# elador/FeatureDetection

Hardware: AMD Instinct MI355X
Metric: Mpatches/s (extract+WVM+SVM) per GPU, 640x480 pyramid (higher is better)
Workload: dtype u8/i32/f32/f64; 1 GPU; config 1/metric config: ffpDetectApp FaceFrontal.cfg five-stage cascade on 640x480 BGR frames: 13-layer pyramid, 20x20 windows step 1 (16185 windows/frame), HistEq64 -> WVM 280 filters -> OE -> RBF-SVM 1024 SV -> NMS; fd_pyramid_update_frames + fd_detect_five_stage_frames (the frames of a call share one pyramid aren...; frames_per_call=64, calls_in_flight=11, parallelism=image-shard dp1

## Files before the change

### featuredetection_amd/csrc/pyramid.hip

```cpp
#include "fd_internal.hpp"
#include <algorithm>
#include <cstring>

namespace {

constexpr int MAXJ = 16;

struct ResizeJob {
    int dw, dh;
    uint32_t dst_off;
    double scale_x, scale_y;
};
struct ResizeJobs {
    int n;
    ResizeJob j[MAXJ];
};
struct DownJob {
    int sw, sh;
    uint32_t src_off, dst_off;
};
struct FusedJob {
    int dw0, dh0, dw1, dh1;
    uint32_t dst0_off;
    uint32_t dst1_off;
    uint32_t xtab;
    double scale_y;
};
struct FusedJobs {
    int n;
    FusedJob j[MAXJ];
};
struct DownJobs {
    int n;
    int tile0[MAXJ + 1];
    DownJob j[MAXJ];
};
struct FilterJob {
    int w, h;
    uint32_t src_off, dst_off;
};
struct FilterJobs {
    int n;
    FilterJob j[MAXJ];
};

__device__ __forceinline__ int reflect101(int p, int len) {
    if (len == 1) return 0;
    while (p < 0 || p >= len) {
        if (p < 0) p = -p;
        else p = 2 * len - 2 - p;
    }
    return p;
}
__device__ __forceinline__ int reflect1(int p, int len) {
    if (len < 3) return reflect101(p, len);
    const int q = p < 0 ? -p : (p >= len ? 2 * len - 2 - p : p);
    return min(max(q, 0), len - 1);
}

struct FramePtrs {
    const uint8_t* p[FD_MAX_FRAMES];
};
__device__ __forceinline__ unsigned int mul24(unsigned int a, unsigned int b) {
    unsigned int r;
    asm("v_mul_u32_u24 %0, %1, %2" : "=v"(r) : "v"(a), "v"(b));
    return r;
}
__device__ __forceinline__ unsigned int mul24_s(unsigned int a_uniform, unsigned int b) {
    unsigned int r;
    asm("v_mul_u32_u24 %0, %1, %2" : "=v"(r) : "s"(a_uniform), "v"(b));
    return r;
}
__device__ __forceinline__ unsigned int mad24(unsigned int a, unsigned int b, unsigned int c) {
    unsigned int r;
    asm("v_mad_u32_u24 %0, %1, %2, %3" : "=v"(r) : "v"(a), "v"(b), "v"(c));
    return r;
}
__device__ __forceinline__ unsigned int mulhi24(unsigned int a, unsigned int b) {
    unsigned int r;
    asm("v_mul_hi_u32_u24 %0, %1, %2" : "=v"(r) : "v"(a), "v"(b));
    return r;
}
typedef unsigned short u16x2 __attribute__((ext_vector_type(2)));
__device__ __forceinline__ uint32_t ld_u32_unaligned(const uint8_t* p) {
    uint32_t v;
    __builtin_memcpy(&v, p, 4);
    return v;
}
__device__ __forceinline__ uint32_t gray_of(uint32_t b, uint32_t g, uint32_t r) { return (b * 1868u + g * 9617u + r * 4899u + 8192u) >> 14; }

__global__ void k_frames_to_gray(FramePtrs frames, uint8_t* __restrict__ grayBase, size_t imageStride, int n, int ch) {
    const uint8_t* __restrict__ src = frames.p[blockIdx.y];
    uint8_t* __restrict__ gray = grayBase + (size_t)blockIdx.y * imageStride;
    const int nq = n >> 2;
    const bool aligned = ((uintptr_t)src & 3) == 0;
    const int stride = gridDim.x * blockDim.x;
    auto load3 = [&](int q, uint32_t (&w)[3]) {
        if (aligned) {
            const uint32_t* s3 = reinterpret_cast<const uint32_t*>(src) + 3 * (size_t)q;
            w[0] = s3[0]; w[1] = s3[1]; w[2] = s3[2];
        } else {
            const uint8_t* s1 = src + 12 * (size_t)q;
            w[0] = ld_u32_unaligned(s1); w[1] = ld_u32_unaligned(s1 + 4); w[2] = ld_u32_unaligned(s1 + 8);
        }
    };
    auto gray4 = [&](const uint32_t (&w)[3]) {
        const uint32_t g0 = gray_of(w[0] & 255u, (w[0] >> 8) & 255u, (w[0] >> 16) & 255u);
        const uint32_t g1 = gray_of(w[0] >> 24, w[1] & 255u, (w[1] >> 8) & 255u);
        const uint32_t g2 = gray_of((w[1] >> 16) & 255u, w[1] >> 24, w[2] & 255u);
        const uint32_t g3 = gray_of((w[2] >> 8) & 255u, (w[2] >> 16) & 255u, w[2] >> 24);
        return g0 | (g1 << 8) | (g2 << 16) | (g3 << 24);
    };
    constexpr int GQ = 4;
    for (int q = blockIdx.x * blockDim.x + threadIdx.x; q < nq; q += GQ * stride) {
        if (ch == 3) {
            uint32_t w[GQ][3];
#pragma unroll
            for (int i = 0; i < GQ; ++i) load3(min(q + i * stride, nq - 1), w[i]);
#pragma unroll
            for (int i = 0; i < GQ; ++i)
                if (q + i * stride < nq) reinterpret_cast<uint32_t*>(gray)[q + i * stride] = gray4(w[i]);
        } else {
            uint32_t w[GQ];
#pragma unroll
            for (int i = 0; i < GQ; ++i) w[i] = ld_u32_unaligned(src + 4 * (size_t)min(q + i * stride, nq - 1));
#pragma unroll
            for (int i = 0; i < GQ; ++i)
                if (q + i * stride < nq) reinterpret_cast<uint32_t*>(gray)[q + i * stride] = w[i];
        }
    }
    if (blockIdx.x == 0 && (int)threadIdx.x < (n & 3)) {
        const int i = (nq << 2) + threadIdx.x;
        gray[i] = ch == 3 ? (uint8_t)gray_of(src[3 * (size_t)i], src[3 * (size_t)i + 1], src[3 * (size_t)i + 2]) : src[i];
    }
}

__global__ void k_bgr2gray(const uint8_t* __restrict__ bgr, uint8_t* __restrict__ gray, int n) {
    int i = blockIdx.x * blockDim.x + threadIdx.x;
    int stride = gridDim.x * blockDim.x;
    for (; i < n; i += stride) {
        int b = bgr[3 * (size_t)i], g = bgr[3 * (size_t)i + 1], r = bgr[3 * (size_t)i + 2];
        gray[i] = (uint8_t)((b * 1868 + g * 9617 + r * 4899 + 8192) >> 14);
// ... 75 lines not shown
    __shared__ int4 rowTab[TL_H];
    const ResizeJob jb = jobs.j[blockIdx.y];
    const uint8_t* src = arena + (size_t)blockIdx.z * imageStride + src_off;
    uint8_t* dst = out + (size_t)blockIdx.z * imageStride + jb.dst_off;
    const int tilesX = (jb.dw + TL_W - 1) / TL_W, tilesY = (jb.dh + TL_H - 1) / TL_H;
    auto srcX = [&](int dx, float& fx) {
        fx = (float)((dx + 0.5) * jb.scale_x - 0.5);
        int sx = (int)floorf(fx);
        fx -= sx;
        if (sx < 0) { fx = 0; sx = 0; }
        if (sx >= sw - 1) { fx = 0; sx = sw - 1; }
        return sx;
    };
    auto srcY = [&](int dy, float& fy) {
        fy = (float)((dy + 0.5) * jb.scale_y - 0.5);
        const int sy = (int)floorf(fy);
        fy -= sy;
        return sy;
    };
    auto clampY = [&](int y) { return y < 0 ? 0 : (y >= sh ? sh - 1 : y); };
    const int c = threadIdx.x & 63, rq = __builtin_amdgcn_readfirstlane(threadIdx.x >> 6);
    for (int t = blockIdx.x; t < tilesX * tilesY; t += gridDim.x) {
        const int ty = t / tilesX, tx = t - ty * tilesX;
        const int dx0 = tx * TL_W, dy0 = ty * TL_H;
        const int X0 = max(0, (int)((float)dx0 * (float)jb.scale_x) - 1), Y0 = max(0, (int)((float)dy0 * (float)jb.scale_y) - 1);
        {
            const int x = X0 + 4 * c;
            const bool colok = c < TL_PITCH / 4;
            uint32_t v[TL_ROWS / 4];
#pragma unroll
            for (int k = 0; k < TL_ROWS / 4; ++k) {
                const int sy = min(Y0 + rq + 4 * k, sh - 1);
                v[k] = 0;
                if (colok && x + 3 < sw) v[k] = ld_u32_unaligned(src + (uint32_t)(sy * sw) + x);
            }
            if (colok && x + 3 >= sw) {
#pragma unroll 1
                for (int k = 0; k < TL_ROWS / 4; ++k) {
                    const uint8_t* row = src + (uint32_t)(min(Y0 + rq + 4 * k, sh - 1) * sw);
                    uint32_t w = 0;
                    for (int b = 0; b < 4; ++b) w |= (uint32_t)row[min(x + b, sw - 1)] << (8 * b);
                    v[k] = w;
                }
            }
            if (colok) {
#pragma unroll
                for (int k = 0; k < TL_ROWS / 4; ++k) *reinterpret_cast<uint32_t*>(&tile[(rq + 4 * k) * TL_PITCH + 4 * c]) = v[k];
            }
        }
        if (threadIdx.x < TL_H) {
            float fy;
            const int sy = srcY(dy0 + threadIdx.x, fy);
            rowTab[threadIdx.x] = make_int4((clampY(sy) - Y0) * TL_PITCH, (clampY(sy + 1) - Y0) * TL_PITCH, __float2int_rn((1.f - fy) * 2048),
                                            __float2int_rn(fy * 2048));
        }
        __syncthreads();
        const int dx = dx0 + c;
        if (dx < jb.dw) {
            float fx;
            const int sx = srcX(dx, fx);
            const int a0 = __float2int_rn((1.f - fx) * 2048), a1 = __float2int_rn(fx * 2048);
            const int lx = sx - X0, lx1 = (sx + 1 < sw ? sx + 1 : sx) - X0;
            uint8_t* dp = dst + (uint32_t)((dy0 + rq * (TL_H / 4)) * jb.dw) + dx;
#pragma unroll
            for (int k = 0; k < TL_H / 4; ++k, dp += jb.dw) {
                const int rr = rq * (TL_H / 4) + k;
                if (dy0 + rr < jb.dh) {
                    const int4 rt = rowTab[rr];
                    const uint8_t* S0 = tile + rt.x;
                    const uint8_t* S1 = tile + rt.y;
                    const unsigned int r0 = __umul24(S0[lx], a0) + __umul24(S0[lx1], a1);
                    const unsigned int r1 = __umul24(S1[lx], a0) + __umul24(S1[lx1], a1);
                    *dp = (uint8_t)(((__umul24(rt.z, r0 >> 4) >> 16) + (__umul24(rt.w, r1 >> 4) >> 16) + 2) >> 2);
                }
            }
        }
        __syncthreads();
    }
}

#ifdef FD_PYR_PROF
constexpr int PYR_PROF_WGS = 65536;
__device__ unsigned long long fd_pyr_prof[PYR_PROF_WGS * 8];
#define PYR_T(x) const unsigned long long x = __builtin_amdgcn_s_memtime()
#else
#define PYR_T(x)
#endif
constexpr int FT_W1 = 62, FT_H1 = 16;
constexpr int G0_W = 2 * FT_W1 + 3, G0_H = 2 * FT_H1 + 3, G0_PITCH = 128;
constexpr int FS_PITCH = 256;
constexpr int FS_LOADS = (2 * G0_H + 3) / 4;
struct FusedFetch {
    uint32_t v[FS_LOADS];
    int2 ex;
    uint32_t taps;
};
__device__ __forceinline__ void fused_issue(FusedFetch& f, const uint8_t* __restrict__ src, int sw, int sh, const int2* __restrict__ tabs,
                                            const FusedJob& jb, const int4 d) {
    const int X0 = d.x, ncol = d.y;
    const int gx0 = 2 * (d.z & 0xffff) * FT_W1 - 2, gy0 = 2 * (int)((uint32_t)d.z >> 16) * FT_H1 - 2;
    const int lane = threadIdx.x & 63, wave = __builtin_amdgcn_readfirstlane(threadIdx.x >> 6);
    uint32_t rowOff;
    {
        const int py = gy0 + min((wave >> 1) + 2 * lane, G0_H - 1), pr = py < 0 ? -py : (py >= jb.dh0 ? 2 * jb.dh0 - 2 - py : py);
        float fy = (float)((min(max(pr, 0), jb.dh0 - 1) + 0.5) * jb.scale_y - 0.5);
        const int sy = (int)floorf(fy);
        fy -= sy;
        f.taps = (uint32_t)__float2int_rn((1.f - fy) * 2048) | (uint32_t)__float2int_rn(fy * 2048) << 16;
        rowOff = mul24((uint32_t)min(max(sy + (wave & 1), 0), sh - 1), (uint32_t)sw);
    }
    const uint32_t voff = (uint32_t)(4 * min(lane, (ncol - 1) >> 2) + X0);
#pragma unroll
    for (int q = 0; q < FS_LOADS; ++q) f.v[q] = ld_u32_unaligned(src + ((uint32_t)__builtin_amdgcn_readlane((int)rowOff, q) + voff));
    f.ex = tabs[jb.xtab + reflect101(gx0 + (int)(threadIdx.x & 127), jb.dw0)];
}

__global__ __launch_bounds__(256) void k_resize_down(uint8_t* __restrict__ arena0, uint32_t src_off, int sw, int sh, const int2* __restrict__ tabs,
                                                     FusedJobs jobs, uint32_t tileTab, int tilesPerFrame, int nimg, size_t imageStride) {
    __shared__ __attribute__((aligned(16))) uint8_t stage[4 * FS_LOADS * FS_PITCH];
    __shared__ __attribute__((aligned(16))) uint8_t g0[G0_H * G0_PITCH];
    __shared__ uint2 taps[G0_H];
    const int4* tiles = reinterpret_cast<const int4*>(tabs + tileTab);
    const int lane = threadIdx.x & 63, wave = __builtin_amdgcn_readfirstlane(threadIdx.x >> 6);
    const bool byXcd = nimg >= 8 && (gridDim.x & 7u) == 0;
    const int xcd = blockIdx.x & 7;
    const int slot = byXcd ? (int)(blockIdx.x >> 3) : (int)blockIdx.x, nslot = byXcd ? (int)(gridDim.x >> 3) : (int)gridDim.x;
    const int items = (byXcd ? (nimg - xcd + 7) >> 3 : nimg) * tilesPerFrame;
    auto frame_of = [&](int item) { const int fi = item / tilesPerFrame; return byXcd ? xcd + 8 * fi : fi; };
    auto desc_of = [&](int item) { return item < items ? tiles[item % tilesPerFrame] : make_int4(0, 0, 0, 0); };

    int item = slot;
    if (item >= items) return;
    int4 d = desc_of(item);
    FusedFetch f;
    fused_issue(f, arena0 + (size_t)frame_of(item) * imageStride + src_off, sw, sh, tabs, jobs.j[d.w], d);
    int itemN = item + nslot;
    int4 dN = desc_of(itemN);

#ifdef FD_PYR_PROF
    unsigned long long pacc[6] = {0, 0, 0, 0, 0, 0}, ptiles = 0;
#endif
    for (; item < items; item = itemN, d = dN, itemN += nslot, dN = desc_of(itemN)) {
        PYR_T(p0);
        const FusedJob jb = jobs.j[d.w];
        uint8_t* arena = arena0 + (size_t)frame_of(item) * imageStride;
        const int X0 = d.x;
        const int x1 = (d.z & 0xffff) * FT_W1, y1 = (int)((uint32_t)d.z >> 16) * FT_H1;
        const int gx0 = 2 * x1 - 2, gy0 = 2 * y1 - 2;
        {
            static_assert(2 * G0_H <= 4 * FS_LOADS && FS_PITCH == 256, "stage holds a dword per lane for slots wave + 4 q");
#pragma unroll
            for (int q = 0; q < FS_LOADS; ++q) *reinterpret_cast<uint32_t*>(&stage[(wave + 4 * q) * FS_PITCH + 4 * lane]) = f.v[q];
            const int i = (wave >> 1) + 2 * lane;
            if ((wave & 1) == 0 && i < G0_H) taps[i] = make_uint2((f.taps & 0xffffu) << 12, (f.taps >> 16) << 12);
        }
        const int2 ex = f.ex;
        PYR_T(p1);
        __syncthreads();
        PYR_T(p2);
        if (itemN < items)
            fused_issue(f, arena0 + (size_t)frame_of(itemN) * imageStride + src_off, sw, sh, tabs, jobs.j[dN.w], dN);
        PYR_T(p3);
        {
            const int c = threadIdx.x & 127, half = __builtin_amdgcn_readfirstlane(threadIdx.x >> 7);
            if (c < G0_W) {
                const int rBase = half * (G0_H - 18);
                const int lx = min(max(ex.x - X0, 0), FS_PITCH - 1) + 2 * rBase * FS_PITCH;
                int lx1 = lx + 1;
                asm("" : "+v"(lx1));
                const uint8_t *sp = stage + lx, *sp1 = stage + lx1;
                const uint2* tp = taps + rBase;
                const u16x2 aw = __builtin_bit_cast(u16x2, ex.y);
                uint8_t* gp = g0 + rBase * G0_PITCH + c;
#pragma unroll
                for (int i = 0; i < 18; ++i) {
                    const uint8_t *s = sp + 2 * i * FS_PITCH, *s1 = sp1 + 2 * i * FS_PITCH;
                    const u16x2 p0 = {s[0], s1[0]}, p1 = {s[FS_PITCH], s1[FS_PITCH]};
                    const uint2 t = tp[i];
                    const unsigned int h0 = __builtin_amdgcn_udot2(p0, aw, 0u, false) & ~15u;
                    const unsigned int h1 = __builtin_amdgcn_udot2(p1, aw, 0u, false) & ~15u;
                    gp[i * G0_PITCH] = (uint8_t)((mulhi24(t.x, h0) + mulhi24(t.y, h1) + 2) >> 2);
                }
            }
        }
        PYR_T(p4);
        __syncthreads();
        PYR_T(p5);
        {
            const int c1 = lane;
            const int x = x1 + c1;
            if (c1 < FT_W1 && x < jb.dw1) {
                constexpr int PR = FT_H1 / 4;
                const uint8_t* T = g0 + (2 * wave * PR) * G0_PITCH + 2 * c1;
                int h[2 * PR + 3];
#pragma unroll
                for (int r = 0; r < 2 * PR + 3; ++r) {
                    const uint8_t* S = T + r * G0_PITCH;
                    const uint32_t p01 = *reinterpret_cast<const uint16_t*>(S), p23 = *reinterpret_cast<const uint16_t*>(S + 2);
                    h[r] = (int)__builtin_amdgcn_udot4(p01 | (p23 << 16), 0x04060401u, (uint32_t)S[4], false);
                }
                uint8_t* dp = arena + jb.dst1_off + (uint32_t)((y1 + wave * PR) * jb.dw1) + x;
#pragma unroll
                for (int j = 0; j < PR; ++j, dp += jb.dw1) {
                    if (y1 + wave * PR + j < jb.dh1) {
                        const int v = h[2 * j + 2] * 6 + (h[2 * j + 1] + h[2 * j + 3]) * 4 + h[2 * j] + h[2 * j + 4];
                        *dp = (uint8_t)((v + 128) >> 8);
                    }
                }
            }
        }
        if (jb.dst0_off != 0xffffffffu) {
            uint8_t* d0 = arena + jb.dst0_off;
            for (int i = threadIdx.x; i < 32 * 128; i += 256) {
                const int r = 2 + (i >> 7), c = 2 + (i & 127);
                const int gx = gx0 + c, gy = gy0 + r;
                if (c < 2 + 2 * FT_W1 && gx < jb.dw0 && gy < jb.dh0) d0[(uint32_t)(gy * jb.dw0) + gx] = g0[r * G0_PITCH + c];
            }
        }
#ifdef FD_PYR_PROF
        {
            const unsigned long long p6 = __builtin_amdgcn_s_memtime();
            pacc[0] += p1 - p0; pacc[1] += p2 - p1; pacc[2] += p3 - p2; pacc[3] += p4 - p3; pacc[4] += p5 - p4; pacc[5] += p6 - p5; ++ptiles;
        }
#endif
    }
#ifdef FD_PYR_PROF
    if (threadIdx.x == 0 && blockIdx.x < (unsigned int)PYR_PROF_WGS) {
        for (int i = 0; i < 6; ++i) fd_pyr_prof[blockIdx.x * 8 + i] = pacc[i];
        fd_pyr_prof[blockIdx.x * 8 + 6] = ptiles;
    }
#endif
}

__device__ __forceinline__ int reflect_cf(int p, int len) {
    int q = p < 0 ? -p : p;
    q = q >= len ? 2 * len - 2 - q : q;
    return min(max(q, 0), len - 1);
}
constexpr int PD_W = 62;
__global__ __launch_bounds__(256) void k_pyrdown_tiled(uint8_t* __restrict__ arena, DownJobs jobs, size_t imageStride) {
    __shared__ __attribute__((aligned(16))) uint8_t tile[TL_ROWS * TL_PITCH];
    arena += (size_t)blockIdx.z * imageStride;
    const int c = threadIdx.x & 63, rq = __builtin_amdgcn_readfirstlane(threadIdx.x >> 6);
    constexpr int NROWS = 2 * PD_TH + 3, PD_LD = (NROWS + 7) / 8;
    static_assert(2 * (3 + 4 * (PD_LD - 1)) + 1 < TL_ROWS && 128 <= TL_PITCH && 2 * PD_W + 3 <= 128, "pyrDown stage");
    for (int g = blockIdx.x; g < jobs.tile0[jobs.n]; g += gridDim.x) {
        int ji = 0;
        while (ji + 1 < jobs.n && g >= jobs.tile0[ji + 1]) ++ji;
        const DownJob jb = jobs.j[ji];
        const int t = g - jobs.tile0[ji];
        const int sw = jb.sw, sh = jb.sh;
        const int dw = (sw + 1) / 2, dh = (sh + 1) / 2;
        const uint8_t* src = arena + jb.src_off;
        uint8_t* dst = arena + jb.dst_off;
        const int tilesX = (dw + PD_W - 1) / PD_W;
        const int ty = t / tilesX, tx = t - ty * tilesX;
        const int dx0 = tx * PD_W, dy0 = ty * PD_TH;
        const int X0 = 2 * dx0 - 2, Y0 = 2 * dy0 - 2;
        {
            const int j4 = 4 * (c & 31), half = c >> 5;
            const int xs = X0 + j4;
            const int xc = min(max(xs, 0), max(sw - 4, 0));
            const uint32_t lastDw = (uint32_t)max(sw * sh - 4, 0);
            uint32_t v[PD_LD];
#pragma unroll
            for (int k = 0; k < PD_LD; ++k) {
                const int r = 2 * (rq + 4 * k) + half;
                v[k] = ld_u32_unaligned(src + min((uint32_t)(reflect_cf(Y0 + r, sh) * sw + xc), lastDw));
            }
            if (X0 < 0 || X0 + 128 > sw) {
                if (!(xs >= 0 && xs + 3 < sw)) {
#pragma unroll
                    for (int k = 0; k < PD_LD; ++k) {
                        const int r = 2 * (rq + 4 * k) + half;
                        const uint8_t* row = src + (uint32_t)(reflect_cf(Y0 + r, sh) * sw);
                        uint32_t w = 0;
#pragma unroll
                        for (int b = 0; b < 4; ++b) w |= (uint32_t)row[reflect_cf(xs + b, sw)] << (8 * b);
                        v[k] = w;
                    }
                }
            }
#pragma unroll
            for (int k = 0; k < PD_LD; ++k) *reinterpret_cast<uint32_t*>(&tile[(2 * (rq + 4 * k) + half) * TL_PITCH + j4]) = v[k];
        }
        __syncthreads();
        const int x = dx0 + c;
        if (c < PD_W && x < dw) {
            constexpr int PR = PD_TH / 4;
            const uint8_t* T = tile + (2 * rq * PR) * TL_PITCH + 2 * c;
            int h[2 * PR + 3];
#pragma unroll
            for (int r = 0; r < 2 * PR + 3; ++r) {
                const uint8_t* S = T + r * TL_PITCH;
                const uint32_t p01 = *reinterpret_cast<const uint16_t*>(S), p23 = *reinterpret_cast<const uint16_t*>(S + 2);
                h[r] = (int)__builtin_amdgcn_udot4(p01 | (p23 << 16), 0x04060401u, (uint32_t)S[4], false);
            }
            uint8_t* dp = dst + (uint32_t)((dy0 + rq * PR) * dw) + x;
#pragma unroll
            for (int j = 0; j < PR; ++j, dp += dw) {
                if (dy0 + rq * PR + j < dh) {
                    const int v = h[2 * j + 2] * 6 + (h[2 * j + 1] + h[2 * j + 3]) * 4 + h[2 * j] + h[2 * j + 4];
                    *dp = (uint8_t)((v + 128) >> 8);
                }
            }
        }
        __syncthreads();
    }
}

__device__ __forceinline__ float grad_pair(const uint8_t* __restrict__ src, int w, int h, int x, int y, int ksize, int& gx, int& gy) {
    if (ksize == 1 || ksize == 3) {
        const int xm = reflect101(x - 1, w), xp = reflect101(x + 1, w);
        const int ym = reflect101(y - 1, h), yp = reflect101(y + 1, h);
        const uint8_t *S0 = src + (size_t)ym * w, *S1 = src + (size_t)y * w, *S2 = src + (size_t)yp * w;
        if (ksize == 1) {
            gx = S1[xp] - S1[xm];
            gy = S2[x] - S0[x];
            return 0.5f;
        }
        gx = (S0[xp] - S0[xm]) + 2 * (S1[xp] - S1[xm]) + (S2[xp] - S2[xm]);
        gy = (S2[xm] - S0[xm]) + 2 * (S2[x] - S0[x]) + (S2[xp] - S0[xp]);
        return 0.125f;
    }
    int a, d1, d2, d3, s0, s1, s2, s3;
    float scale;
    if (ksize == 5) { a = 2; d1 = 2; d2 = 1; d3 = 0; s0 = 6; s1 = 4; s2 = 1; s3 = 0; scale = 1.f / 128.f; }
    else if (ksize == 7) { a = 3; d1 = 5; d2 = 4; d3 = 1; s0 = 20; s1 = 15; s2 = 6; s3 = 1; scale = 1.f / 2048.f; }
    else { a = 1; d1 = 1; d2 = 0; d3 = 0; s0 = 10; s1 = 3; s2 = 0; s3 = 0; scale = 1.f / 32.f; }
// ... 203 lines not shown
    __shared__ unsigned int lm[4][3];
#pragma unroll
    for (int c = 0; c < 3; ++c) {
        unsigned long long sc = s[c];
        unsigned int mc = m[c];
        for (int o = 32; o > 0; o >>= 1) {
            sc += __shfl_down(sc, o, 64);
            mc = max(mc, (unsigned int)__shfl_down((int)mc, o, 64));
        }
        if ((threadIdx.x & 63) == 0) { ls[threadIdx.x >> 6][c] = sc; lm[threadIdx.x >> 6][c] = mc; }
    }
    __syncthreads();
    if (threadIdx.x < 3) {
        const int c = threadIdx.x;
        atomicAdd(&stats[blockIdx.y].sum[c], ls[0][c] + ls[1][c] + ls[2][c] + ls[3][c]);
        atomicMax(&stats[blockIdx.y].max[c], max(max(lm[0][c], lm[1][c]), max(lm[2][c], lm[3][c])));
    }
}

__global__ __launch_bounds__(256) void k_gw_gray(FramePtrs frames, const GwStats* __restrict__ stats, uint8_t* __restrict__ grayBase,
                                                 size_t imageStride, int n) {
    __shared__ double scale[3];
    __shared__ uint32_t tab[3][256];
    const uint8_t* __restrict__ src = frames.p[blockIdx.y];
    uint8_t* __restrict__ gray = grayBase + (size_t)blockIdx.y * imageStride;
    const int nq = n >> 2;
    const bool aligned = ((uintptr_t)src & 3) == 0;
    const int stride = gridDim.x * blockDim.x;
    int q = blockIdx.x * blockDim.x + threadIdx.x;
    uint32_t w[GW_GQ][3] = {};
    if (q < nq) {
#pragma unroll
        for (int i = 0; i < GW_GQ; ++i) gw_load3(src, aligned, min(q + i * stride, nq - 1), w[i]);
    }
    if (threadIdx.x < 64) {
        const GwStats& S = stats[blockIdx.y];
        double mean[3], maxNew[3];
        for (int c = 0; c < 3; ++c) { mean[c] = (double)S.sum[c] / n; maxNew[c] = (uint8_t)S.max[c] / mean[c]; }
        double mx = maxNew[0];
        if (maxNew[1] > mx) mx = maxNew[1];
        if (maxNew[2] > mx) mx = maxNew[2];
        if (threadIdx.x == 0)
            for (int c = 0; c < 3; ++c) scale[c] = 255.0 / (mean[c] * mx);
    }
    __syncthreads();
    {
        const uint32_t v = threadIdx.x;
        const uint32_t wgt[3] = {1868u, 9617u, 4899u};
#pragma unroll
        for (int c = 0; c < 3; ++c) {
            const int r = __double2int_rn(scale[c] * (double)v);
            tab[c][v] = (uint32_t)min(255, max(0, r)) * wgt[c] + (c == 0 ? 8192u : 0u);
        }
    }
    __syncthreads();
    auto gray1 = [&](uint32_t b, uint32_t g, uint32_t r) { return (tab[0][b] + tab[1][g] + tab[2][r]) >> 14; };
    auto gray4 = [&](const uint32_t (&x)[3]) {
        const uint32_t g0 = gray1(x[0] & 255u, (x[0] >> 8) & 255u, (x[0] >> 16) & 255u);
        const uint32_t g1 = gray1(x[0] >> 24, x[1] & 255u, (x[1] >> 8) & 255u);
        const uint32_t g2 = gray1((x[1] >> 16) & 255u, x[1] >> 24, x[2] & 255u);
        const uint32_t g3 = gray1((x[2] >> 8) & 255u, (x[2] >> 16) & 255u, x[2] >> 24);
        return g0 | (g1 << 8) | (g2 << 16) | (g3 << 24);
    };
    while (q < nq) {
        const int qn = q + GW_GQ * stride;
        uint32_t wn[GW_GQ][3] = {};
        if (qn < nq) {
#pragma unroll
            for (int i = 0; i < GW_GQ; ++i) gw_load3(src, aligned, min(qn + i * stride, nq - 1), wn[i]);
        }
#pragma unroll
        for (int i = 0; i < GW_GQ; ++i)
            if (q + i * stride < nq) reinterpret_cast<uint32_t*>(gray)[q + i * stride] = gray4(w[i]);
#pragma unroll
        for (int i = 0; i < GW_GQ; ++i) { w[i][0] = wn[i][0]; w[i][1] = wn[i][1]; w[i][2] = wn[i][2]; }
        q = qn;
    }
    if (blockIdx.x == 0 && (int)threadIdx.x < (n & 3)) {
        const size_t i = ((size_t)nq << 2) + threadIdx.x;
        gray[i] = (uint8_t)gray1(src[3 * i], src[3 * i + 1], src[3 * i + 2]);
    }
}

inline uint32_t align256(size_t v) { return (uint32_t)((v + 255) & ~(size_t)255); }

void build_gradient_lut(int bins, bool signedGradients, bool interpolate, std::vector<uint8_t>& lut) {
    const double PI = 3.1415926535897932384626433832795;
    const int E = interpolate ? 4 : 2;
    lut.resize((size_t)65536 * E);
    for (int x = 0; x < 256; ++x) {
        double gradientX = ((double)x - 127) / 255;
        for (int y = 0; y < 256; ++y) {
            double gradientY = ((double)y - 127) / 255;
            double direction = std::atan2(gradientY, gradientX);
            double magnitude = std::sqrt(gradientX * gradientX + gradientY * gradientY);
            double bin;
            if (signedGradients) {
                direction += PI;
                bin = direction * bins / (2 * PI);
            } else {
                if (direction < 0) direction += PI;
                bin = direction * bins / PI;
            }
            auto sat = [](double v) { int r = fd_cvRound(v); return (uint8_t)(r < 0 ? 0 : (r > 255 ? 255 : r)); };
            size_t index = (size_t)x | ((size_t)y << 8);
            if (!interpolate) {
                lut[2 * index] = (uint8_t)((uint8_t)std::round(bin) % (unsigned)bins);
                lut[2 * index + 1] = sat(255 * magnitude);
            } else {
                uint8_t w1 = sat(255 * magnitude * (bin - std::floor(bin)));
                lut[4 * index] = (uint8_t)((uint8_t)std::floor(bin) % (unsigned)bins);
                lut[4 * index + 1] = sat(255 * magnitude - w1);
                lut[4 * index + 2] = (uint8_t)((uint8_t)std::ceil(bin) % (unsigned)bins);
                lut[4 * index + 3] = w1;
            }
        }
    }
}

void build_resize_tables(fd_pyramid* p, int W, int H) {
    p->rtab_x.assign(p->all.size(), ~0u);
    static const int mode = [] { const char* e = getenv("FD_PYR_FUSED"); return e ? atoi(e) : 1; }();
    if (mode == 0) return;
    std::vector<int2> tab;
    std::vector<std::vector<int4>> tiles;
    p->rtile_off.clear();
    p->rtile_cnt.clear();
    int nfused = 0;
    for (size_t k = 0; k + 1 < p->all.size(); ++k) {
        const HostLayer& L = p->all[k];
        const HostLayer& D = p->all[k + 1];
        if (L.depth != 0 || D.depth != 1 || D.chain != L.chain) continue;
        if (L.w == W && L.h == H && L.gray_off == p->gray_full_off) continue;
        if (L.w < 3 || L.h < 3 || W > 65535 || H > 65535) continue;
        if (L.kept && mode != 2) continue;
        const double scale_x = 1. / ((double)L.w / W);
        std::vector<int2> xt((size_t)L.w);
        for (int dx = 0; dx < L.w; ++dx) {
            float fx = (float)((dx + 0.5) * scale_x - 0.5);
            int sx = (int)floorf(fx);
            fx -= sx;
            if (sx < 0) { fx = 0; sx = 0; }
            if (sx >= W - 1) { fx = 0; sx = W - 1; }
            const int a0 = (int)nearbyintf((1.f - fx) * 2048), a1 = (int)nearbyintf(fx * 2048);
            xt[(size_t)dx] = make_int2(sx, a0 | (a1 << 16));
        }
        bool fits = true;
        for (int x1 = 0; x1 < D.w && fits; x1 += FT_W1) {
            const int cLo = std::max(0, 2 * x1 - 2), cHi = std::min(L.w - 1, 2 * x1 - 2 + G0_W - 1);
            fits = std::min(W - 1, xt[(size_t)cHi].x + 1) - xt[(size_t)cLo].x + 1 <= FS_PITCH;
        }
        if (!fits) continue;
        {
            if (nfused % MAXJ == 0) tiles.emplace_back();
            std::vector<int4>& tl = tiles.back();
            for (int ty = 0; ty * FT_H1 < D.h; ++ty)
                for (int tx = 0; tx * FT_W1 < D.w; ++tx) {
                    const int gx0 = 2 * tx * FT_W1 - 2;
                    const int cLo = std::max(0, gx0), cHi = std::min(L.w - 1, gx0 + G0_W - 1);
                    const int X0 = xt[(size_t)cLo].x, ncol = std::min(W - 1, xt[(size_t)cHi].x + 1) - X0 + 1;
                    tl.push_back(make_int4(X0, ncol, (int)((uint32_t)tx | (uint32_t)ty << 16), nfused % MAXJ));
                }
            ++nfused;
        }
        p->rtab_x[k] = (uint32_t)tab.size();
        tab.insert(tab.end(), xt.begin(), xt.end());
    }
    if (tab.empty()) return;
    for (const std::vector<int4>& tl : tiles) {
        if (tab.size() & 1) tab.push_back(make_int2(0, 0));
        p->rtile_off.push_back((uint32_t)tab.size());
        p->rtile_cnt.push_back((int)tl.size());
        for (const int4& t : tl) { tab.push_back(make_int2(t.x, t.y)); tab.push_back(make_int2(t.z, t.w)); }
    }
    p->rtab.reserve(sizeof(int2) * tab.size());
    HIP_CHECK(hipMemcpy(p->rtab.p, tab.data(), sizeof(int2) * tab.size(), hipMemcpyHostToDevice));
}

void build_layout(fd_pyramid* p, int W, int H) {
    p->img_w = W;
    p->img_h = H;
    p->all.clear();
    p->kept.clear();
    size_t off = 0;
    p->gray_full_off = 0;
    off = align256((size_t)W * H);
    const int fch = p->filter_kind == FD_LAYER_GRADBIN ? (p->interpolate ? 4 : 2) : 1;
    for (size_t i = 0; i < p->octl; ++i) {
        double scaleFactor = std::pow(p->inc, (double)i);
        int w = fd_cvRound(W * scaleFactor), h = fd_cvRound(H * scaleFactor);
        if (w < 1 || h < 1) FD_THROW(FD_ERR_INVALID_ARGUMENT, "ImagePyramid: layer %zu would be empty", i);
        int depth = 0;
        const bool isFull = (w == W && h == H);
        HostLayer L{(int)i, scaleFactor, w, h, 1, (uint32_t)(isFull ? p->gray_full_off : off), 0, scaleFactor <= p->maxS && scaleFactor >= p->minS, (int)i, depth};
        if (!isFull) off = align256(off + (size_t)w * h);
        p->all.push_back(L);
        int pw = w, ph = h;
        scaleFactor *= 0.5;
        for (size_t j = 1; scaleFactor >= p->minS && pw > 1; ++j, scaleFactor *= 0.5) {
            int dw = (pw + 1) / 2, dh = (ph + 1) / 2;
            HostLayer D{(int)(i + j * p->octl), scaleFactor, dw, dh, 1, (uint32_t)off, 0, scaleFactor <= p->maxS, (int)i, (int)j};
            off = align256(off + (size_t)dw * dh);
            p->all.push_back(D);
            pw = dw;
            ph = dh;
        }
    }
    for (size_t k = 0; k < p->all.size(); ++k) {
        HostLayer& L = p->all[k];
        if (!L.kept) continue;
        L.ch = fch;
        if (p->filter_kind == FD_LAYER_NONE) L.filt_off = L.gray_off;
        else {
            L.filt_off = (uint32_t)off;
            off = align256(off + (size_t)L.w * L.h * fch);
            if (p->filter_kind == FD_LAYER_GRADBIN && p->grad_blur > 0) {
                L.blur_off = (uint32_t)off;
                off = align256(off + (size_t)L.w * L.h);
            }
        }
        p->kept.push_back((int)k);
    }
    if (off > 0xfffffff0ull) FD_THROW(FD_ERR_INVALID_ARGUMENT, "ImagePyramid: pyramid exceeds 4 GB arena");
    std::sort(p->kept.begin(), p->kept.end(), [&](int a, int b) { return p->all[a].index < p->all[b].index; });
    p->arena_bytes = off + 256;
    p->image_stride = (p->arena_bytes + 255) & ~(size_t)255;
    if (p->nimg > 1 && p->image_stride * (size_t)p->nimg > 0xfffffff0ull * 16) FD_THROW(FD_ERR_INVALID_ARGUMENT, "ImagePyramid: multi-frame pyramid too large");
    p->arena.reserve(p->image_stride * (size_t)p->nimg);
    p->h_layer_table.clear();
    for (int k : p->kept) {
        const HostLayer& L = p->all[k];
        p->h_layer_table.push_back(LayerDesc{L.w, L.h, L.ch, 0, L.gray_off, L.filt_off});
    }
    p->layer_table.reserve(sizeof(LayerDesc) * std::max<size_t>(1, p->h_layer_table.size()));
    if (!p->h_layer_table.empty())
        HIP_CHECK(hipMemcpyAsync(p->layer_table.p, p->h_layer_table.data(), sizeof(LayerDesc) * p->h_layer_table.size(),
                                 hipMemcpyHostToDevice, p->ctx->stream));
    build_resize_tables(p, W, H);
}

int grid_for(int npix) { return std::max(1, std::min(1024, (npix + 255) / 256)); }
int tile_grid_for(int ntiles) { return std::max(1, std::min(1024, ntiles)); }

void pyramid_update(fd_pyramid* p, const uint8_t* image, int W, int H, int ch, int is_device, hipStream_t st, const uint8_t* const* frames = nullptr) {
    if (!image && !frames) FD_THROW(FD_ERR_INVALID_ARGUMENT, "fd_pyramid_update: image is NULL");
    if (p->nimg > 1 && !frames) FD_THROW(FD_ERR_INVALID_ARGUMENT, "fd_pyramid_update: the pyramid holds %d frames, use fd_pyramid_update_frames", p->nimg);
    if (p->nimg > 1 && p->filter_kind != FD_LAYER_NONE) FD_THROW(FD_ERR_INVALID_ARGUMENT, "multi-frame pyramids have no layer filters");
    if (W < 1 || H < 1) FD_THROW(FD_ERR_INVALID_ARGUMENT, "fd_pyramid_update: empty image");
    if (ch != 1 && ch != 3) FD_THROW(FD_ERR_INVALID_ARGUMENT, "fd_pyramid_update: image must have 1 or 3 channels");
    const bool greyworld = p->image_filter != FD_IMAGE_GRAY;
    if (greyworld && ch != 3) FD_THROW(FD_ERR_INVALID_ARGUMENT, "GreyWorldNormalizationFilter: The image type must be CV_8UC3");
    if (greyworld && (size_t)W * H > 0x7fffffffull) FD_THROW(FD_ERR_INVALID_ARGUMENT, "GreyWorldNormalizationFilter: image too large");
    if (W != p->img_w || H != p->img_h || p->all.empty()) build_layout(p, W, H);
    uint8_t* arena = p->arena.as<uint8_t>();
    const size_t npix = (size_t)W * H;
    const int NI = frames ? p->nimg : 1;
    const size_t IS = p->image_stride;
    auto enqueue_rest = [&]() {
    int maxDepth = 0;
    for (const HostLayer& L : p->all) maxDepth = std::max(maxDepth, L.depth);
    {
        ResizeJobs jobs;
        jobs.n = 0;
        int maxpix = 0, maxtiles = 0;
        auto flush = [&]() {
            if (!jobs.n) return;
            bool fits = true;
            for (int q = 0; q < jobs.n; ++q)
                fits = fits && jobs.j[q].scale_x >= 1.0 && jobs.j[q].scale_x <= 2.05 && jobs.j[q].scale_y >= 1.0 && jobs.j[q].scale_y <= 2.05;
            if (fits)
                hipLaunchKernelGGL(k_resize_tiled, dim3(tile_grid_for(maxtiles), jobs.n, NI), dim3(256), 0, st, arena, arena, p->gray_full_off, W, H, jobs, IS);
            else
                hipLaunchKernelGGL(k_resize_linear, dim3(grid_for(maxpix), jobs.n, NI), dim3(256), 0, st, arena, arena, p->gray_full_off, W, H, jobs, IS);
            jobs.n = 0;
            maxpix = 0;
            maxtiles = 0;
        };
        for (size_t k = 0; k < p->all.size(); ++k) {
            const HostLayer& L = p->all[k];
            if (L.depth != 0) continue;
            if (L.w == W && L.h == H && L.gray_off == p->gray_full_off) continue;
            if (p->rtab_x[k] != ~0u) continue;
            ResizeJob& j = jobs.j[jobs.n++];
            j.dw = L.w; j.dh = L.h; j.dst_off = L.gray_off;
            j.scale_x = 1. / ((double)L.w / W);
            j.scale_y = 1. / ((double)L.h / H);
            maxpix = std::max(maxpix, L.w * L.h);
            maxtiles = std::max(maxtiles, ((L.w + TL_W - 1) / TL_W) * ((L.h + TL_H - 1) / TL_H));
            if (jobs.n == MAXJ) flush();
        }
        flush();
    }
    {
        FusedJobs jobs;
        jobs.n = 0;
        size_t group = 0;
        auto flush = [&]() {
            if (!jobs.n) return;
            static int perCu = 0;
            if (perCu == 0 && (hipOccupancyMaxActiveBlocksPerMultiprocessor(&perCu, k_resize_down, 256, 0) != hipSuccess || perCu < 1)) perCu = 4;
            const int tilesPerFrame = p->rtile_cnt[group];
            int grid = (int)std::min<int64_t>((int64_t)tilesPerFrame * NI, (int64_t)p->ctx->num_cus * perCu);
            if (NI >= 8 && grid >= 64) grid &= ~7;
            hipLaunchKernelGGL(k_resize_down, dim3(grid), dim3(256), 0, st, arena, p->gray_full_off, W, H, p->rtab.as<int2>(), jobs, p->rtile_off[group], tilesPerFrame, NI, IS);
            jobs.n = 0;
            ++group;
        };
        for (size_t k = 0; k + 1 < p->all.size(); ++k) {
            if (p->rtab_x[k] == ~0u) continue;
            const HostLayer& L = p->all[k];
            const HostLayer& D = p->all[k + 1];
            FusedJob& j = jobs.j[jobs.n++];
            j.dw0 = L.w; j.dh0 = L.h; j.dw1 = D.w; j.dh1 = D.h;
            j.dst0_off = (L.kept && L.gray_off != p->gray_full_off) ? L.gray_off : 0xffffffffu;
            j.dst1_off = D.gray_off;
            j.xtab = p->rtab_x[k];
            j.scale_y = 1. / ((double)L.h / H);
            if (jobs.n == MAXJ) flush();
        }
        flush();
    }
    {
        DownJobs dj;
        dj.n = 0;
        dj.tile0[0] = 0;
        auto flush1 = [&]() {
            if (!dj.n) return;
            hipLaunchKernelGGL(k_pyrdown_tiled, dim3(tile_grid_for(dj.tile0[dj.n]), 1, NI), dim3(256), 0, st, arena, dj, IS);
            dj.n = 0;
        };
        for (size_t k = 1; k < p->all.size(); ++k) {
            const HostLayer& L = p->all[k];
            if (L.depth != 1 || p->rtab_x[k - 1] != ~0u) continue;
            const HostLayer& S = p->all[k - 1];
            DownJob& j = dj.j[dj.n++];
            j.sw = S.w; j.sh = S.h; j.src_off = S.gray_off; j.dst_off = L.gray_off;
            dj.tile0[dj.n] = dj.tile0[dj.n - 1] + ((L.w + PD_W - 1) / PD_W) * ((L.h + PD_TH - 1) / PD_TH);
            if (dj.n == MAXJ) flush1();
        }
        flush1();
    }
    for (int d = 2; d <= maxDepth; ++d) {
        DownJobs jobs;
        jobs.n = 0;
        jobs.tile0[0] = 0;
        auto flush = [&]() {
            if (!jobs.n) return;
            hipLaunchKernelGGL(k_pyrdown_tiled, dim3(tile_grid_for(jobs.tile0[jobs.n]), 1, NI), dim3(256), 0, st, arena, jobs, IS);
            jobs.n = 0;
        };
        for (size_t k = 0; k < p->all.size(); ++k) {
            const HostLayer& L = p->all[k];
            if (L.depth != d) continue;
            const HostLayer& S = p->all[k - 1];
            DownJob& j = jobs.j[jobs.n++];
            j.sw = S.w; j.sh = S.h; j.src_off = S.gray_off; j.dst_off = L.gray_off;
            jobs.tile0[jobs.n] = jobs.tile0[jobs.n - 1] + ((L.w + PD_W - 1) / PD_W) * ((L.h + PD_TH - 1) / PD_TH);
            if (jobs.n == MAXJ) flush();
        }
        flush();
    }
    if (p->filter_kind != FD_LAYER_NONE) {
        FilterJobs jobs, bjobs;
        jobs.n = 0;
        bjobs.n = 0;
        int maxpix = 0;
        const bool blur = p->filter_kind == FD_LAYER_GRADBIN && p->grad_blur > 0;
        auto flush = [&]() {
            if (!jobs.n) return;
            dim3 g(grid_for(maxpix), jobs.n);
            if (blur) hipLaunchKernelGGL(k_box_blur, g, dim3(256), 0, st, arena, p->grad_blur, bjobs);
            bjobs.n = 0;
            if (p->filter_kind == FD_LAYER_GRADBIN) {
                if (p->interpolate)
                    hipLaunchKernelGGL(k_gradbin<4>, g, dim3(256), 0, st, arena, p->lut.as<uint8_t>(), p->grad_kernel, jobs);
                else
                    hipLaunchKernelGGL(k_gradbin<2>, g, dim3(256), 0, st, arena, p->lut.as<uint8_t>(), p->grad_kernel, jobs);
            } else {
                hipLaunchKernelGGL(k_lbp, g, dim3(256), 0, st, arena, p->lbp_type, jobs);
            }
            jobs.n = 0;
            maxpix = 0;
        };
        for (int k : p->kept) {
            const HostLayer& L = p->all[k];
            FilterJob& j = jobs.j[jobs.n++];
            j.w = L.w; j.h = L.h; j.src_off = blur ? L.blur_off : L.gray_off; j.dst_off = L.filt_off;
            if (blur) {
                FilterJob& b = bjobs.j[bjobs.n++];
                b.w = L.w; b.h = L.h; b.src_off = L.gray_off; b.dst_off = L.blur_off;
            }
            maxpix = std::max(maxpix, L.w * L.h);
            if (jobs.n == MAXJ) flush();
        }
        flush();
    }
    };
    auto enqueue_greyworld_gray = [&](const FramePtrs& fp) {
        GwStats* stats = p->gw_stats.as<GwStats>();
        HIP_CHECK(hipMemsetAsync(stats, 0, sizeof(GwStats) * (size_t)NI, st));
        const int cus = std::max(1, p->ctx->num_cus);
        const int perFrame = std::max(1, std::min(cus, 4 * cus / NI));
        const int gx = std::max(1, std::min((int)((npix / 4 + 1023) / 1024), perFrame));
        hipLaunchKernelGGL(k_gw_stats, dim3(gx, NI), dim3(256), 0, st, fp, stats, (int)npix);
        hipLaunchKernelGGL(k_gw_gray, dim3(gx, NI), dim3(256), 0, st, fp, stats, arena + p->gray_full_off, IS, (int)npix);
    };
    if (frames) {
        FramePtrs fp;
        if (!is_device) {
            p->input.reserve(npix * ch * (size_t)NI);
            for (int f = 0; f < NI; ++f) {
                HIP_CHECK(hipMemcpyAsync(p->input.as<uint8_t>() + (size_t)f * npix * ch, frames[f], npix * ch, hipMemcpyHostToDevice, st));
                fp.p[f] = p->input.as<uint8_t>() + (size_t)f * npix * ch;
            }
        } else {
            for (int f = 0; f < NI; ++f) fp.p[f] = frames[f];
        }
        if (greyworld) enqueue_greyworld_gray(fp);
        else
            hipLaunchKernelGGL(k_frames_to_gray, dim3(grid_for((int)(npix / 16 + 1)), NI), dim3(256), 0, st, fp, arena + p->gray_full_off, IS, (int)npix, ch);
    } else {
        const uint8_t* dimg = image;
        if (!is_device) {
            p->input.reserve(npix * ch);
            HIP_CHECK(hipMemcpyAsync(p->input.p, image, npix * ch, hipMemcpyHostToDevice, st));
            dimg = p->input.as<uint8_t>();
        }
        if (greyworld) {
            FramePtrs fp{};
            fp.p[0] = dimg;
            enqueue_greyworld_gray(fp);
// ... 397 lines not shown
```

Baseline: 3773 Mpatches/s.

## Fold full-res pyrDown into fused resize kernel and XCD-map pyrDown launches

Adds a copy-tile mode to the fused resize+pyrDown kernel. The full-resolution level's first pyrDown now runs inside that kernel as extra tiles that copy source pixels straight into the g0 stage, so it no longer needs a separate k_pyrdown_tiled launch. It also changes k_pyrdown_tiled to a flat grid that groups frames by XCD, so each chiplet works on the same frames and keeps them local in its L2. The costs are more branching in the fused kernel, larger tile lists, and a persistent-style indexing change whose grid size now scales with the frame count.

```diff
diff --git a/featuredetection_amd/csrc/pyramid.hip b/featuredetection_amd/csrc/pyramid.hip
--- a/featuredetection_amd/csrc/pyramid.hip
+++ b/featuredetection_amd/csrc/pyramid.hip
@@ -1,6 +1,14 @@
 #include "fd_internal.hpp"
 #include <algorithm>
+#include <atomic>
 #include <cstring>
+
+#ifndef FD_PYR_XCD
+#define FD_PYR_XCD 1
+#endif
+#ifndef FD_PYR_COPY
+#define FD_PYR_COPY 1
+#endif
 
 namespace {
 
@@ -58,6 +66,12 @@
     return min(max(q, 0), len - 1);
 }
 
+__device__ __forceinline__ int reflect_cf(int p, int len) {
+    int q = p < 0 ? -p : p;
+    q = q >= len ? 2 * len - 2 - q : q;
+    return min(max(q, 0), len - 1);
+}
+
 struct FramePtrs {
     const uint8_t* p[FD_MAX_FRAMES];
 };
@@ -299,7 +313,7 @@
 #ifdef FD_PYR_PROF
 constexpr int PYR_PROF_WGS = 65536;
 __device__ unsigned long long fd_pyr_prof[PYR_PROF_WGS * 8];
-#define PYR_T(x) const unsigned long long x = __builtin_amdgcn_s_memtime()
+#define PYR_T(x) x = __builtin_amdgcn_s_memtime()
 #else
 #define PYR_T(x)
 #endif
@@ -332,6 +346,29 @@
     f.ex = tabs[jb.xtab + reflect101(gx0 + (int)(threadIdx.x & 127), jb.dw0)];
 }
 
+constexpr int FT_COPY = 0x100;
+constexpr int CP_LOADS = (G0_H + 7) / 8;
+static_assert(CP_LOADS <= FS_LOADS && G0_PITCH == 128 && G0_W <= G0_PITCH, "a copy tile's rows are 32 dwords of g0");
+__device__ __forceinline__ void copy_issue(FusedFetch& f, const uint8_t* __restrict__ src, int sw, int sh, const int4 d) {
+    const int gx0 = 2 * (d.z & 0xffff) * FT_W1 - 2, gy0 = 2 * (int)((uint32_t)d.z >> 16) * FT_H1 - 2;
+    const int j4 = 4 * (threadIdx.x & 31), r0 = threadIdx.x >> 5;
+    const int xs = gx0 + j4;
+    const int xc = min(max(xs, 0), max(sw - 4, 0));
+    const uint32_t lastDw = (uint32_t)max(sw * sh - 4, 0);
+#pragma unroll
+    for (int k = 0; k < CP_LOADS; ++k) {
+        const int r = min(r0 + 8 * k, G0_H - 1);
+        f.v[k] = ld_u32_unaligned(src + min((uint32_t)(reflect_cf(gy0 + r, sh) * sw + xc), lastDw));
+    }
+    if (gx0 < 0 || gx0 + G0_PITCH > sw) {
+        uint32_t sel = 0;
+#pragma unroll
+        for (int b = 0; b < 4; ++b) sel |= (uint32_t)min(max(reflect_cf(xs + b, sw) - xc, 0), 3) << (8 * b);
+#pragma unroll
+        for (int k = 0; k < CP_LOADS; ++k) f.v[k] = __builtin_amdgcn_perm(f.v[k], f.v[k], sel);
+    }
+}
+
 __global__ __launch_bounds__(256) void k_resize_down(uint8_t* __restrict__ arena0, uint32_t src_off, int sw, int sh, const int2* __restrict__ tabs,
                                                      FusedJobs jobs, uint32_t tileTab, int tilesPerFrame, int nimg, size_t imageStride) {
     __shared__ __attribute__((aligned(16))) uint8_t stage[4 * FS_LOADS * FS_PITCH];
@@ -350,53 +387,69 @@
     if (item >= items) return;
     int4 d = desc_of(item);
     FusedFetch f;
-    fused_issue(f, arena0 + (size_t)frame_of(item) * imageStride + src_off, sw, sh, tabs, jobs.j[d.w], d);
+    auto issue = [&](int it, const int4 dd) {
+        const uint8_t* src = arena0 + (size_t)frame_of(it) * imageStride + src_off;
+        if (dd.w & FT_COPY) copy_issue(f, src, sw, sh, dd);
+        else fused_issue(f, src, sw, sh, tabs, jobs.j[dd.w], dd);
+    };
+    issue(item, d);
     int itemN = item + nslot;
     int4 dN = desc_of(itemN);
 
 #ifdef FD_PYR_PROF
     unsigned long long pacc[6] = {0, 0, 0, 0, 0, 0}, ptiles = 0;
+    unsigned long long p0 = 0, p1 = 0, p2 = 0, p3 = 0, p4 = 0, p5 = 0;
 #endif
     for (; item < items; item = itemN, d = dN, itemN += nslot, dN = desc_of(itemN)) {
         PYR_T(p0);
-        const FusedJob jb = jobs.j[d.w];
+        const FusedJob jb = jobs.j[d.w & (FT_COPY - 1)];
         uint8_t* arena = arena0 + (size_t)frame_of(item) * imageStride;
         const int X0 = d.x;
         const int x1 = (d.z & 0xffff) * FT_W1, y1 = (int)((uint32_t)d.z >> 16) * FT_H1;
         const int gx0 = 2 * x1 - 2, gy0 = 2 * y1 - 2;
-        {
-            static_assert(2 * G0_H <= 4 * FS_LOADS && FS_PITCH == 256, "stage holds a dword per lane for slots wave + 4 q");
-#pragma unroll
-            for (int q = 0; q < FS_LOADS; ++q) *reinterpret_cast<uint32_t*>(&stage[(wave + 4 * q) * FS_PITCH + 4 * lane]) = f.v[q];
-            const int i = (wave >> 1) + 2 * lane;
-            if ((wave & 1) == 0 && i < G0_H) taps[i] = make_uint2((f.taps & 0xffffu) << 12, (f.taps >> 16) << 12);
-        }
-        const int2 ex = f.ex;
-        PYR_T(p1);
-        __syncthreads();
-        PYR_T(p2);
-        if (itemN < items)
-            fused_issue(f, arena0 + (size_t)frame_of(itemN) * imageStride + src_off, sw, sh, tabs, jobs.j[dN.w], dN);
-        PYR_T(p3);
-        {
-            const int c = threadIdx.x & 127, half = __builtin_amdgcn_readfirstlane(threadIdx.x >> 7);
-            if (c < G0_W) {
-                const int rBase = half * (G0_H - 18);
-                const int lx = min(max(ex.x - X0, 0), FS_PITCH - 1) + 2 * rBase * FS_PITCH;
-                int lx1 = lx + 1;
-                asm("" : "+v"(lx1));
-                const uint8_t *sp = stage + lx, *sp1 = stage + lx1;
-                const uint2* tp = taps + rBase;
-                const u16x2 aw = __builtin_bit_cast(u16x2, ex.y);
-                uint8_t* gp = g0 + rBase * G0_PITCH + c;
-#pragma unroll
-                for (int i = 0; i < 18; ++i) {
-                    const uint8_t *s = sp + 2 * i * FS_PITCH, *s1 = sp1 + 2 * i * FS_PITCH;
-                    const u16x2 p0 = {s[0], s1[0]}, p1 = {s[FS_PITCH], s1[FS_PITCH]};
-                    const uint2 t = tp[i];
-                    const unsigned int h0 = __builtin_amdgcn_udot2(p0, aw, 0u, false) & ~15u;
-                    const unsigned int h1 = __builtin_amdgcn_udot2(p1, aw, 0u, false) & ~15u;
-                    gp[i * G0_PITCH] = (uint8_t)((mulhi24(t.x, h0) + mulhi24(t.y, h1) + 2) >> 2);
+        if (d.w & FT_COPY) {
+            PYR_T(p1);
+            __syncthreads();
+            PYR_T(p2);
+            const int j4 = 4 * (threadIdx.x & 31), r0 = threadIdx.x >> 5;
+#pragma unroll
+            for (int k = 0; k < CP_LOADS; ++k) *reinterpret_cast<uint32_t*>(&g0[min(r0 + 8 * k, G0_H - 1) * G0_PITCH + j4]) = f.v[k];
+            if (itemN < items) issue(itemN, dN);
+            PYR_T(p3);
+        } else {
+            {
+                static_assert(2 * G0_H <= 4 * FS_LOADS && FS_PITCH == 256, "stage holds a dword per lane for slots wave + 4 q");
+#pragma unroll
+                for (int q = 0; q < FS_LOADS; ++q) *reinterpret_cast<uint32_t*>(&stage[(wave + 4 * q) * FS_PITCH + 4 * lane]) = f.v[q];
+                const int i = (wave >> 1) + 2 * lane;
+                if ((wave & 1) == 0 && i < G0_H) taps[i] = make_uint2((f.taps & 0xffffu) << 12, (f.taps >> 16) << 12);
+            }
+            const int2 ex = f.ex;
+            PYR_T(p1);
+            __syncthreads();
+            PYR_T(p2);
+            if (itemN < items) issue(itemN, dN);
+            PYR_T(p3);
+            {
+                const int c = threadIdx.x & 127, half = __builtin_amdgcn_readfirstlane(threadIdx.x >> 7);
+                if (c < G0_W) {
+                    const int rBase = half * (G0_H - 18);
+                    const int lx = min(max(ex.x - X0, 0), FS_PITCH - 1) + 2 * rBase * FS_PITCH;
+                    int lx1 = lx + 1;
+                    asm("" : "+v"(lx1));
+                    const uint8_t *sp = stage + lx, *sp1 = stage + lx1;
+                    const uint2* tp = taps + rBase;
+                    const u16x2 aw = __builtin_bit_cast(u16x2, ex.y);
+                    uint8_t* gp = g0 + rBase * G0_PITCH + c;
+#pragma unroll
+                    for (int i = 0; i < 18; ++i) {
+                        const uint8_t *s = sp + 2 * i * FS_PITCH, *s1 = sp1 + 2 * i * FS_PITCH;
+                        const u16x2 p0 = {s[0], s1[0]}, p1 = {s[FS_PITCH], s1[FS_PITCH]};
+                        const uint2 t = tp[i];
+                        const unsigned int h0 = __builtin_amdgcn_udot2(p0, aw, 0u, false) & ~15u;
+                        const unsigned int h1 = __builtin_amdgcn_udot2(p1, aw, 0u, false) & ~15u;
+                        gp[i * G0_PITCH] = (uint8_t)((mulhi24(t.x, h0) + mulhi24(t.y, h1) + 2) >> 2);
+                    }
                 }
             }
         }
@@ -449,19 +502,19 @@
 #endif
 }
 
-__device__ __forceinline__ int reflect_cf(int p, int len) {
-    int q = p < 0 ? -p : p;
-    q = q >= len ? 2 * len - 2 - q : q;
-    return min(max(q, 0), len - 1);
-}
 constexpr int PD_W = 62;
-__global__ __launch_bounds__(256) void k_pyrdown_tiled(uint8_t* __restrict__ arena, DownJobs jobs, size_t imageStride) {
+__global__ __launch_bounds__(256) void k_pyrdown_tiled(uint8_t* __restrict__ arena0, DownJobs jobs, size_t imageStride, int nimgXcd) {
     __shared__ __attribute__((aligned(16))) uint8_t tile[TL_ROWS * TL_PITCH];
-    arena += (size_t)blockIdx.z * imageStride;
+    const int ntile = jobs.tile0[jobs.n];
+    const int xcd = blockIdx.x & 7;
+    const int items = nimgXcd ? ((nimgXcd - xcd + 7) >> 3) * ntile : ntile;
+    const int step = nimgXcd ? (int)(gridDim.x >> 3) : (int)gridDim.x;
     const int c = threadIdx.x & 63, rq = __builtin_amdgcn_readfirstlane(threadIdx.x >> 6);
     constexpr int NROWS = 2 * PD_TH + 3, PD_LD = (NROWS + 7) / 8;
     static_assert(2 * (3 + 4 * (PD_LD - 1)) + 1 < TL_ROWS && 128 <= TL_PITCH && 2 * PD_W + 3 <= 128, "pyrDown stage");
-    for (int g = blockIdx.x; g < jobs.tile0[jobs.n]; g += gridDim.x) {
+    for (int item = nimgXcd ? (int)(blockIdx.x >> 3) : (int)blockIdx.x; item < items; item += step) {
+        const int fi = nimgXcd ? item / ntile : 0, g = item - fi * ntile;
+        uint8_t* arena = arena0 + (size_t)(nimgXcd ? xcd + 8 * fi : (int)blockIdx.z) * imageStride;
         int ji = 0;
         while (ji + 1 < jobs.n && g >= jobs.tile0[ji + 1]) ++ji;
         const DownJob jb = jobs.j[ji];
@@ -831,6 +884,7 @@
     }
 }
 
+constexpr uint32_t RTAB_COPY = 0xfffffffeu;
 inline uint32_t align256(size_t v) { return (uint32_t)((v + 255) & ~(size_t)255); }
 
 void build_gradient_lut(int bins, bool signedGradients, bool interpolate, std::vector<uint8_t>& lut) {
@@ -876,11 +930,12 @@
     p->rtile_off.clear();
     p->rtile_cnt.clear();
     int nfused = 0;
+    size_t copyK = ~(size_t)0;
     for (size_t k = 0; k + 1 < p->all.size(); ++k) {
         const HostLayer& L = p->all[k];
         const HostLayer& D = p->all[k + 1];
         if (L.depth != 0 || D.depth != 1 || D.chain != L.chain) continue;
-        if (L.w == W && L.h == H && L.gray_off == p->gray_full_off) continue;
+        if (L.w == W && L.h == H && L.gray_off == p->gray_full_off) { copyK = k; continue; }
         if (L.w < 3 || L.h < 3 || W > 65535 || H > 65535) continue;
         if (L.kept && mode != 2) continue;
         const double scale_x = 1. / ((double)L.w / W);
@@ -916,6 +971,13 @@
         tab.insert(tab.end(), xt.begin(), xt.end());
     }
     if (tab.empty()) return;
+    if (FD_PYR_COPY && copyK != ~(size_t)0 && W >= 4 && W <= 65535 && H <= 65535) {
+        const HostLayer& D = p->all[copyK + 1];
+        if (nfused % MAXJ == 0) tiles.emplace_back();
+        for (int ty = 0; ty * FT_H1 < D.h; ++ty)
+            for (int tx = 0; tx * FT_W1 < D.w; ++tx) tiles.back().push_back(make_int4(0, 0, (int)((uint32_t)tx | (uint32_t)ty << 16), (nfused % MAXJ) | FT_COPY));
+        p->rtab_x[copyK] = RTAB_COPY;
+    }
     for (const std::vector<int4>& tl : tiles) {
         if (tab.size() & 1) tab.push_back(make_int2(0, 0));
         p->rtile_off.push_back((uint32_t)tab.size());
@@ -1046,8 +1108,12 @@
         size_t group = 0;
         auto flush = [&]() {
             if (!jobs.n) return;
-            static int perCu = 0;
-            if (perCu == 0 && (hipOccupancyMaxActiveBlocksPerMultiprocessor(&perCu, k_resize_down, 256, 0) != hipSuccess || perCu < 1)) perCu = 4;
+            static std::atomic<int> perCuOnce{0};
+            int perCu = perCuOnce.load(std::memory_order_relaxed);
+            if (perCu == 0) {
+                if (hipOccupancyMaxActiveBlocksPerMultiprocessor(&perCu, k_resize_down, 256, 0) != hipSuccess || perCu < 1) perCu = 4;
+                perCuOnce.store(perCu, std::memory_order_relaxed);
+            }
             const int tilesPerFrame = p->rtile_cnt[group];
             int grid = (int)std::min<int64_t>((int64_t)tilesPerFrame * NI, (int64_t)p->ctx->num_cus * perCu);
             if (NI >= 8 && grid >= 64) grid &= ~7;
@@ -1055,27 +1121,40 @@
             jobs.n = 0;
             ++group;
         };
-        for (size_t k = 0; k + 1 < p->all.size(); ++k) {
-            if (p->rtab_x[k] == ~0u) continue;
-            const HostLayer& L = p->all[k];
-            const HostLayer& D = p->all[k + 1];
-            FusedJob& j = jobs.j[jobs.n++];
-            j.dw0 = L.w; j.dh0 = L.h; j.dw1 = D.w; j.dh1 = D.h;
-            j.dst0_off = (L.kept && L.gray_off != p->gray_full_off) ? L.gray_off : 0xffffffffu;
-            j.dst1_off = D.gray_off;
-            j.xtab = p->rtab_x[k];
-            j.scale_y = 1. / ((double)L.h / H);
-            if (jobs.n == MAXJ) flush();
-        }
+        for (int pass = 0; pass < 2; ++pass)
+            for (size_t k = 0; k + 1 < p->all.size(); ++k) {
+                if (p->rtab_x[k] == ~0u || (p->rtab_x[k] == RTAB_COPY) != (pass == 1)) continue;
+                const HostLayer& L = p->all[k];
+                const HostLayer& D = p->all[k + 1];
+                FusedJob& j = jobs.j[jobs.n++];
+                j.dw0 = L.w; j.dh0 = L.h; j.dw1 = D.w; j.dh1 = D.h;
+                j.dst0_off = (L.kept && L.gray_off != p->gray_full_off) ? L.gray_off : 0xffffffffu;
+                j.dst1_off = D.gray_off;
+                j.xtab = pass ? 0 : p->rtab_x[k];
+                j.scale_y = 1. / ((double)L.h / H);
+                if (jobs.n == MAXJ) flush();
+            }
         flush();
     }
+    auto launch_down = [&](const DownJobs& dj) {
+        const int ntile = dj.tile0[dj.n];
+        if (FD_PYR_XCD && NI >= 8) {
+            int64_t perXcd = (int64_t)(NI / 8) * ntile;
+#ifdef FD_PYR_XCD_PERSIST
+            perXcd = std::min<int64_t>(perXcd, (int64_t)FD_PYR_XCD_PERSIST * p->ctx->num_cus / 8);
+#endif
+            hipLaunchKernelGGL(k_pyrdown_tiled, dim3((unsigned)(8 * perXcd)), dim3(256), 0, st, arena, dj, IS, NI);
+        } else {
+            hipLaunchKernelGGL(k_pyrdown_tiled, dim3(tile_grid_for(ntile), 1, NI), dim3(256), 0, st, arena, dj, IS, 0);
+        }
+    };
     {
         DownJobs dj;
         dj.n = 0;
         dj.tile0[0] = 0;
         auto flush1 = [&]() {
             if (!dj.n) return;
-            hipLaunchKernelGGL(k_pyrdown_tiled, dim3(tile_grid_for(dj.tile0[dj.n]), 1, NI), dim3(256), 0, st, arena, dj, IS);
+            launch_down(dj);
             dj.n = 0;
         };
         for (size_t k = 1; k < p->all.size(); ++k) {
@@ -1095,7 +1174,7 @@
         jobs.tile0[0] = 0;
         auto flush = [&]() {
             if (!jobs.n) return;
-            hipLaunchKernelGGL(k_pyrdown_tiled, dim3(tile_grid_for(jobs.tile0[jobs.n]), 1, NI), dim3(256), 0, st, arena, jobs, IS);
+            launch_down(jobs);
             jobs.n = 0;
         };
         for (size_t k = 0; k < p->all.size(); ++k) {
```

Result: no change. 3767 Mpatches/s (-0.2%).
